# SiyuanHuang95/SUG

Measured on AMD Instinct MI355X. Metric: point-clouds/sec (train step, N=1024), higher is better.
Workload: dtype f32

## Files before the change

sug_amd/csrc/knn_pc.hip:

```cpp
#include <float.h>
#include "common.h"
#include "mfma_tile.h"


namespace {
using namespace sug_tile;

constexpr int SROW = 36;


__device__ __forceinline__ unsigned lds_addr(const float* p) {
  return (unsigned)(uintptr_t)(const __attribute__((address_space(3))) float*)p;
}

template <int KP>
__device__ __forceinline__ void insert_key_hi(int (&L)[KP], int x) {
#pragma unroll
  for (int u = KP - 1; u >= KP / 2; --u) asm volatile("v_med3_i32 %0, %1, %2, %0" : "+v"(L[u]) : "v"(x), "v"(L[u - 1]));
}
template <int KP>
__device__ __forceinline__ void insert_key_lo(int (&L)[KP], int x) {
#pragma unroll
  for (int u = KP / 2 - 1; u >= 1; --u) asm volatile("v_med3_i32 %0, %1, %2, %0" : "+v"(L[u]) : "v"(x), "v"(L[u - 1]));
  asm volatile("v_min_i32 %0, %0, %1" : "+v"(L[0]) : "v"(x));
}

template <int CP>
__device__ __forceinline__ float exact_dot(const float* __restrict__ a, const float* __restrict__ b) {
  float acc = 0.f;
  if constexpr (CP == 4) {
    acc = fmaf(a[0], b[0], acc); acc = fmaf(a[1], b[1], acc); acc = fmaf(a[2], b[2], acc);
  } else {
    for (int e = 0; e < CP; e += 4) {
      const float4 av = *reinterpret_cast<const float4*>(a + e), bv = *reinterpret_cast<const float4*>(b + e);
      acc = fmaf(av.x, bv.x, acc); acc = fmaf(av.y, bv.y, acc); acc = fmaf(av.z, bv.z, acc); acc = fmaf(av.w, bv.w, acc);
    }
  }
  return acc;
}
template <int CP>
__device__ __forceinline__ float exact_norm(const float* __restrict__ r) {
  if constexpr (CP == 4) {
    return sq3(r[0], r[1], r[2]);
  } else {
    constexpr int CH = CP / 8;
    float pc[CH];
#pragma unroll
    for (int c = 0; c < CH; ++c) {
      const float4 a = *reinterpret_cast<const float4*>(r + 8 * c), b = *reinterpret_cast<const float4*>(r + 8 * c + 4);
      float p = __fmul_rn(a.x, a.x);
      p = fmaf(a.y, a.y, p); p = fmaf(a.z, a.z, p); p = fmaf(a.w, a.w, p);
      p = fmaf(b.x, b.x, p); p = fmaf(b.y, b.y, p); p = fmaf(b.z, b.z, p); p = fmaf(b.w, b.w, p);
      pc[c] = p;
    }
#pragma unroll
    for (int o = 1; o < CH; o <<= 1)
#pragma unroll
      for (int c = 0; c < CH; c += 2 * o) pc[c] = pc[c] + pc[c + o];
    return pc[0];
  }
}

template <int CP, int K, int NP, int NC>
__global__ __launch_bounds__(64 * (NP + NC), 2) void knn_pc_kernel(const float* __restrict__ x, int64_t ldx, int B, int N,
                                                                   int k, int32_t* __restrict__ idx, int force) {
  constexpr int RS = CP + 4;
  constexpr int HALF = CP / 2;
  constexpr int NTP = 64 * NP;
  constexpr int QB = 64 * NC;
  constexpr int QP = QB / NP;
  static_assert(QP == 32 || QP == 64, "a producer wave scores one or two 32-query column blocks");
  extern __shared__ __attribute__((aligned(16))) unsigned char smem[];
  float* s_tile = reinterpret_cast<float*>(smem);
  float* s_norm = s_tile + 3 * TJ * RS;
  float* s_score = s_norm + 4 * TJ;

  const int nq = (N + QB - 1) / QB;
  int b, qb;
  if ((B & 7) == 0) {
    const int grp = blockIdx.x / (8 * nq), rem = blockIdx.x % (8 * nq);
    b = grp * 8 + (rem & 7);
    qb = rem >> 3;
  } else {
    b = blockIdx.x / nq;
    qb = blockIdx.x % nq;
  }
  const float* xb = x + (int64_t)b * N * ldx;
  const int wave = (int)(threadIdx.x >> 6);
  const bool producer = wave < NP;
  const int lane = threadIdx.x & 63;
  const int wv = producer ? wave : wave - NP;
  const int ptid = (int)threadIdx.x;
  const int qj = lane & 31, h = lane >> 5;
  const int q0 = qb * QB;

  const int ntile = (N + TJ - 1) / TJ;
  auto tbuf = [&](int t) { return s_tile + (t % 3) * TJ * RS; };
  auto nbuf = [&](int t) { return s_norm + (t % 3) * TJ; };

  if (producer) {
    TileRegs<CP, NTP> tr;
    tile_load<CP, NTP>(tr, xb, ldx, N, 0, ptid);
    float bq0[HALF], bq1[HALF];
    {
      const int r0 = min(q0 + wv * QP + qj, N - 1), r1 = min(q0 + wv * QP + 32 + qj, N - 1);
      const float* p0 = xb + (int64_t)r0 * ldx;
      const float* p1 = xb + (int64_t)r1 * ldx;
      if constexpr (CP == 4) {
        const float x0 = p0[0], y0 = p0[1], z0 = p0[2], x1 = p1[0], y1 = p1[1], z1 = p1[2];
        bq0[0] = -2.f * (h ? y0 : x0); bq0[1] = h ? 0.f : -2.f * z0;
        bq1[0] = -2.f * (h ? y1 : x1); bq1[1] = h ? 0.f : -2.f * z1;
      } else {
#pragma unroll
        for (int g = 0; g < HALF / 4; ++g) {
          const float4 a = *reinterpret_cast<const float4*>(p0 + h * HALF + 4 * g);
          const float4 c = *reinterpret_cast<const float4*>(p1 + h * HALF + 4 * g);
          bq0[4 * g] = -2.f * a.x; bq0[4 * g + 1] = -2.f * a.y; bq0[4 * g + 2] = -2.f * a.z; bq0[4 * g + 3] = -2.f * a.w;
          bq1[4 * g] = -2.f * c.x; bq1[4 * g + 1] = -2.f * c.y; bq1[4 * g + 2] = -2.f * c.z; bq1[4 * g + 3] = -2.f * c.w;
        }
#pragma unroll
        for (int e = 0; e < HALF; e += 2) {
          const auto u = __builtin_amdgcn_permlane32_swap(__float_as_uint(bq0[e]), __float_as_uint(bq0[e + 1]), false, false);
          bq0[e] = __uint_as_float(u[0]); bq0[e + 1] = __uint_as_float(u[1]);
          const auto v = __builtin_amdgcn_permlane32_swap(__float_as_uint(bq1[e]), __float_as_uint(bq1[e + 1]), false, false);
          bq1[e] = __uint_as_float(v[0]); bq1[e + 1] = __uint_as_float(v[1]);
        }
      }
    }
    auto breg = [](int s2) constexpr { return CP == 4 ? s2 : (s2 < HALF / 2 ? 2 * s2 : 2 * (s2 - HALF / 2) + 1); };

    auto produce = [&](int t, int buf, auto&& mid) {
      const float* arow = tbuf(t) + qj * RS + h * HALF;
      f32x16 acc0, acc1;
#pragma unroll
      for (int r = 0; r < 16; ++r) { acc0[r] = 0.f; acc1[r] = 0.f; }
      if constexpr (CP == 4) {
        const float2 a2 = *reinterpret_cast<const float2*>(arow);
        acc0 = __builtin_amdgcn_mfma_f32_32x32x2f32(a2.x, bq0[0], acc0, 0, 0, 0);
        if constexpr (QP == 64) acc1 = __builtin_amdgcn_mfma_f32_32x32x2f32(a2.x, bq1[0], acc1, 0, 0, 0);
        acc0 = __builtin_amdgcn_mfma_f32_32x32x2f32(a2.y, bq0[1], acc0, 0, 0, 0);
        if constexpr (QP == 64) acc1 = __builtin_amdgcn_mfma_f32_32x32x2f32(a2.y, bq1[1], acc1, 0, 0, 0);
        mid();
      } else {
#pragma unroll
        for (int g = 0; g < HALF / 4; ++g) {
          if (g == HALF / 8) mid();
          const float4 a4 = *reinterpret_cast<const float4*>(arow + 4 * g);
          acc0 = __builtin_amdgcn_mfma_f32_32x32x2f32(a4.x, bq0[breg(4 * g + 0)], acc0, 0, 0, 0);
          if constexpr (QP == 64) acc1 = __builtin_amdgcn_mfma_f32_32x32x2f32(a4.x, bq1[breg(4 * g + 0)], acc1, 0, 0, 0);
          acc0 = __builtin_amdgcn_mfma_f32_32x32x2f32(a4.y, bq0[breg(4 * g + 1)], acc0, 0, 0, 0);
          if constexpr (QP == 64) acc1 = __builtin_amdgcn_mfma_f32_32x32x2f32(a4.y, bq1[breg(4 * g + 1)], acc1, 0, 0, 0);
          acc0 = __builtin_amdgcn_mfma_f32_32x32x2f32(a4.z, bq0[breg(4 * g + 2)], acc0, 0, 0, 0);
          if constexpr (QP == 64) acc1 = __builtin_amdgcn_mfma_f32_32x32x2f32(a4.z, bq1[breg(4 * g + 2)], acc1, 0, 0, 0);
          acc0 = __builtin_amdgcn_mfma_f32_32x32x2f32(a4.w, bq0[breg(4 * g + 3)], acc0, 0, 0, 0);
          if constexpr (QP == 64) acc1 = __builtin_amdgcn_mfma_f32_32x32x2f32(a4.w, bq1[breg(4 * g + 3)], acc1, 0, 0, 0);
        }
      }
      float* d0 = s_score + ((buf * QB + wv * QP) + qj) * SROW + 4 * h;
#pragma unroll
      for (int g = 0; g < 4; ++g)
        *reinterpret_cast<float4*>(d0 + 8 * g) = make_float4(acc0[4 * g], acc0[4 * g + 1], acc0[4 * g + 2], acc0[4 * g + 3]);
      if constexpr (QP == 64) {
        float* d1 = d0 + 32 * SROW;
#pragma unroll
        for (int g = 0; g < 4; ++g)
          *reinterpret_cast<float4*>(d1 + 8 * g) = make_float4(acc1[4 * g], acc1[4 * g + 1], acc1[4 * g + 2], acc1[4 * g + 3]);
      }
    };

    tile_store<CP, true, NTP>(tr, tbuf(0), nbuf(0), N, 0, ptid);
    if (ntile > 1) tile_load<CP, NTP>(tr, xb, ldx, N, TJ, ptid);
    __syncthreads();
    produce(0, 0, [] {});
    if (ntile > 1) tile_store<CP, true, NTP>(tr, tbuf(1), nbuf(1), N, TJ, ptid);
    if (ntile > 2) tile_load<CP, NTP>(tr, xb, ldx, N, 2 * TJ, ptid);
    __syncthreads();
    for (int t = 0; t < ntile; ++t) {
      auto stage = [&] {
        if (t + 2 < ntile) tile_store<CP, true, NTP>(tr, tbuf(t + 2), nbuf(t + 2), N, (t + 2) * TJ, ptid);
        if (t + 3 < ntile) tile_load<CP, NTP>(tr, xb, ldx, N, (t + 3) * TJ, ptid);
      };
      if (t + 1 < ntile) produce(t + 1, (t + 1) & 1, [] {});
      stage();
      __syncthreads();
    }
  } else {
    __builtin_amdgcn_s_setprio(1);
    const float ni = exact_norm<CP>(xb + (int64_t)min(q0 + wv * 64 + lane, N - 1) * ldx);

    constexpr int KP = K + 2;
    constexpr int EMPTY = 0x7fffffff;
    int L[KP];
#pragma unroll
    for (int t = 0; t < KP; ++t) L[t] = EMPTY;
    const int q = q0 + wv * 64 + lane;
    const int idb = N > 1 ? 32 - __clz(N - 1) : 0;
    const int idm = (1 << idb) - 1, nidm = ~idm;
    const unsigned FXMAX = (1u << (31 - idb)) - 2u;
    float scale = 1.f, inv_scale = 1.f;
    float thr = -FLT_MAX;

    auto score = [&](float inner, float nj) { return __fsub_rn(__fsub_rn(-nj, inner), ni); };

    __syncthreads();
    __syncthreads();
    for (int t = 0; t < ntile; ++t) {
      const float* srow = s_score + (((t & 1) * QB + wv * 64) + lane) * SROW;
      const float* nrm = nbuf(t);
      unsigned int mask = 0u;
      if (t == 0) {
        float smin = INFINITY;
#pragma unroll
        for (int g = 0; g < 8; ++g) {
          const float4 s4 = *reinterpret_cast<const float4*>(srow + 4 * g);
          const float4 n4 = *reinterpret_cast<const float4*>(nrm + 4 * g);
          const float sx = score(s4.x, n4.x), sy = score(s4.y, n4.y), sz = score(s4.z, n4.z), sw = score(s4.w, n4.w);
          mask = mask + mask + (sx >= thr ? 1u : 0u);
          mask = mask + mask + (sy >= thr ? 1u : 0u);
          mask = mask + mask + (sz >= thr ? 1u : 0u);
          mask = mask + mask + (sw >= thr ? 1u : 0u);
          smin = fminf(smin, sx >= thr ? sx : INFINITY);
          smin = fminf(smin, sy >= thr ? sy : INFINITY);
          smin = fminf(smin, sz >= thr ? sz : INFINITY);
          smin = fminf(smin, sw >= thr ? sw : INFINITY);
        }
        float R = (smin < 0.f && smin > -FLT_MAX) ? -smin : 1.f;
        scale = (float)FXMAX / R;
        inv_scale = R / (float)FXMAX;
        if (!(scale < FLT_MAX) || !(inv_scale > 0.f)) { scale = 1.f; inv_scale = 1.f; }
      } else {
        const float thr2 = thr == -FLT_MAX ? -FLT_MAX : __fsub_rn(__fadd_rn(thr, ni), 2.4e-7f * (fabsf(thr) + fabsf(ni)));
        unsigned int rej = 0u;
#pragma unroll
        for (int g = 0; g < 8; ++g) {
          const float4 s4 = *reinterpret_cast<const float4*>(srow + 4 * g);
          const float4 n4 = *reinterpret_cast<const float4*>(nrm + 4 * g);
          const float wx = __fsub_rn(__fsub_rn(-n4.x, s4.x), thr2), wy = __fsub_rn(__fsub_rn(-n4.y, s4.y), thr2);
          const float wz = __fsub_rn(__fsub_rn(-n4.z, s4.z), thr2), ww = __fsub_rn(__fsub_rn(-n4.w, s4.w), thr2);
          rej = __builtin_amdgcn_alignbit(rej, __float_as_uint(wx), 31);
          rej = __builtin_amdgcn_alignbit(rej, __float_as_uint(wy), 31);
          rej = __builtin_amdgcn_alignbit(rej, __float_as_uint(wz), 31);
          rej = __builtin_amdgcn_alignbit(rej, __float_as_uint(ww), 31);
        }
        mask = ~rej;
      }
      const int pc = __popc(mask);
      unsigned long long cand = ~0ull;
      int nit = 0;
#pragma unroll
      for (int bit = 5; bit >= 0; --bit) {
        const unsigned long long m = __ballot((pc >> bit) & 1) & cand;
        if (m) {
          nit |= 1 << bit;
          cand = m;
        }
      }
      const unsigned srow_a = lds_addr(srow), nrm_a = lds_addr(nrm);
      float dotA, njA, dotB, njB;
      bool vA, vB;
      int cA, cB;
      auto fetch_issue = [&](float& dot, float& nj, bool& valid, int& c) {
        valid = mask != 0u;
        c = valid ? __builtin_clz(mask) : 0;
        mask &= ~(0x80000000u >> c);
        asm volatile("ds_read_b32 %0, %2\n\tds_read_b32 %1, %3" : "=&v"(dot), "=&v"(nj) : "v"(srow_a + 4u * c), "v"(nrm_a + 4u * c));
      };
      auto fetch_finish = [&](float& dot, float& nj, bool valid, int c, int& key_out) {
        asm volatile("s_waitcnt lgkmcnt(2)" : "+v"(dot), "+v"(nj));
        const unsigned fx = min(__float2uint_rz(-score(dot, nj) * scale), FXMAX);
        key_out = valid ? (int)((fx << idb) | (unsigned)(t * TJ + c)) : EMPTY;
      };
      int key_cur, key_nxt;
      fetch_issue(dotA, njA, vA, cA);
      fetch_issue(dotB, njB, vB, cB);
      fetch_finish(dotA, njA, vA, cA, key_cur);
      for (int it = 0; it < nit; it += 2) {
        fetch_issue(dotA, njA, vA, cA);
        insert_key_hi<KP>(L, key_cur);
        fetch_finish(dotB, njB, vB, cB, key_nxt);
        insert_key_lo<KP>(L, key_cur);
        if (it + 1 < nit) {
          fetch_issue(dotB, njB, vB, cB);
          insert_key_hi<KP>(L, key_nxt);
          fetch_finish(dotA, njA, vA, cA, key_cur);
          insert_key_lo<KP>(L, key_nxt);
        }
      }
      asm volatile("s_waitcnt lgkmcnt(0)" : "+v"(dotA), "+v"(njA), "+v"(dotB), "+v"(njB));
      const int lk = L[KP - 1];
      thr = lk == EMPTY ? -FLT_MAX : -((float)((lk >> idb) + 3) * inv_scale * 1.000002f);
      __syncthreads();
    }

    bool amb = false;
#pragma unroll
    for (int u = 0; u < K; ++u) amb |= ((L[u] ^ L[u + 1]) & nidm) == 0 && L[u] != EMPTY;
    bool rescan = amb && ((L[K - 1] ^ L[KP - 1]) & nidm) == 0 && L[KP - 1] != EMPTY;
    if (force >= 1) amb = true;
    if (force >= 2) rescan = true;
    if (q >= N) amb = rescan = false;
    int32_t* o = idx + ((int64_t)b * N + (q < N ? q : 0)) * k;
    if (q < N && !amb) {
#pragma unroll
      for (int t = 0; t < K; ++t)
        if (t < k) o[t] = L[t] == EMPTY ? q : (L[t] & idm);
    }
    if (__ballot(amb) != 0ull) {
      int* s_keys = reinterpret_cast<int*>(s_score + (0 * QB + wv * 64) * SROW);
      float* s_fv = s_score + (1 * QB + wv * 64) * SROW;
#pragma unroll
      for (int t = 0; t < KP; ++t) s_keys[lane * KP + t] = L[t];
      unsigned long long todo = __ballot(amb && !rescan);
      while (todo) {
        const int ql = __builtin_ctzll(todo);
        todo &= todo - 1;
        const int qi = q0 + wv * 64 + ql;
        const float niq = __shfl(ni, ql);
        const int key = lane < KP ? s_keys[ql * KP + lane] : EMPTY;
        const bool has = key != EMPTY;
        const int j = has ? (key & idm) : 0;
        const float* xq = xb + (int64_t)qi * ldx;
        const float* xj = xb + (int64_t)j * ldx;
        const float dj = exact_dot<CP>(xj, xq);
        const float nj = exact_norm<CP>(xj);
        const float sc = has ? __fsub_rn(__fsub_rn(-nj, __fmul_rn(-2.0f, dj)), niq) : -INFINITY;
        int rank = 0;
#pragma unroll
        for (int v = 0; v < KP; ++v) {
          const float sv = __int_as_float(__builtin_amdgcn_readlane(__float_as_int(sc), v));
          const int jv = __builtin_amdgcn_readlane(has ? j : 0x7fffffff, v);
          rank += (sv > sc || (sv == sc && jv < j)) ? 1 : 0;
        }
        const int nhas = __popcll(__ballot(has));
        int32_t* oq = idx + ((int64_t)b * N + qi) * k;
        if (has && rank < k) oq[rank] = j;
        if (lane < k && lane >= nhas) oq[lane] = qi;
      }
      if (rescan) {
        int* s_fid = s_keys;
        const float* xq = xb + (int64_t)q * ldx;
        for (int t = 0; t < K; ++t) { s_fv[t * 64 + lane] = -INFINITY; s_fid[t * 64 + lane] = q; }
        for (int j = 0; j < N; ++j) {
          const float* xj = xb + (int64_t)j * ldx;
          const float sc = __fsub_rn(__fsub_rn(-exact_norm<CP>(xj), __fmul_rn(-2.0f, exact_dot<CP>(xj, xq))), ni);
          if (sc > s_fv[(K - 1) * 64 + lane]) {
            int u = K - 1;
            while (u > 0 && sc > s_fv[(u - 1) * 64 + lane]) {
              s_fv[u * 64 + lane] = s_fv[(u - 1) * 64 + lane];
              s_fid[u * 64 + lane] = s_fid[(u - 1) * 64 + lane];
              --u;
            }
            s_fv[u * 64 + lane] = sc;
            s_fid[u * 64 + lane] = j;
          }
        }
        for (int t = 0; t < K; ++t)
          if (t < k) o[t] = s_fid[t * 64 + lane];
      }
    }
  }
}

template <int CP, int K, int NP, int NC>
int launch_pc_form(const float* x, int64_t ldx, int B, int N, int k, int32_t* idx, hipStream_t st) {
  constexpr int RS = CP + 4;
  constexpr int QB = 64 * NC;
  const size_t sh = (size_t)(3 * TJ * RS + 4 * TJ + 2 * QB * SROW) * sizeof(float);
  static SugLdsOptIn note;
  if (int rc = sug_allow_dynamic_lds(note, &knn_pc_kernel<CP, K, NP, NC>, (int)sh, "sug_knn(mfma, producer/consumer)")) return rc;
  dim3 grid(sug_divup(N, QB) * B);
  const char* fe = getenv("SUG_KNN_FORCE");
  hipLaunchKernelGGL((knn_pc_kernel<CP, K, NP, NC>), grid, dim3(64 * (NP + NC)), sh, st, x, ldx, B, N, k, idx, fe ? atoi(fe) : 0);
  SUG_LAUNCH_CHECK("sug_knn(mfma, producer/consumer)");
  return SUG_OK;
}

template <int CP, int K>
int launch_pc(const float* x, int64_t ldx, int B, int N, int k, int32_t* idx, hipStream_t st) {
  static const int forced = getenv("SUG_KNN_PW") ? atoi(getenv("SUG_KNN_PW")) : 0;
  const int ncu = sug_cu_count();
  const int64_t grid4 = (int64_t)B * sug_divup(N, 256);
  const bool small = 2 * grid4 <= ncu;
  const int form = (forced == 4 || forced == 44) ? 44 : (forced == 2 || forced == 22) ? 22 : forced == 42 ? 42
                   : !small ? 44 : (CP >= 64 ? 42 : 22);
  if (form == 22) return launch_pc_form<CP, K, 2, 2>(x, ldx, B, N, k, idx, st);
  if (form == 42) return launch_pc_form<CP, K, 4, 2>(x, ldx, B, N, k, idx, st);
  return launch_pc_form<CP, K, 4, 4>(x, ldx, B, N, k, idx, st);
}

template <int K>
int dispatch_pc(const float* x, int64_t ldx, int B, int N, int C, int k, int32_t* idx, hipStream_t st) {
  if (C == 3) return launch_pc<4, K>(x, ldx, B, N, k, idx, st);
  if (C == 64) return launch_pc<64, K>(x, ldx, B, N, k, idx, st);
  return launch_pc<128, K>(x, ldx, B, N, k, idx, st);
}

}

int sug_knn_pc_supported(const float* x, int64_t ldx, int C, int k) {
  if (k > 20) return 0;
  if (C == 3) return 1;
  if (C != 64 && C != 128) return 0;
  return ((uintptr_t)x % 16 == 0) && (ldx % 4 == 0);
}

int sug_knn_pc(const float* x, int64_t ldx, int B, int N, int C, int k, int32_t* idx, hipStream_t st) {
  if (k <= 16) return dispatch_pc<16>(x, ldx, B, N, C, k, idx, st);
  return dispatch_pc<20>(x, ldx, B, N, C, k, idx, st);
}
```

Measured before the change: 13610.

## Fold neighbour norm into MFMA accumulation and use ballot-driven consumer loop

Adds an MF variant in which the producer scales the query by +2 and folds the negated neighbour norm into the score accumulator with one extra rank-1 MFMA. Consumers then read only the fused score, dropping the per-candidate norm LDS loads and one subtraction. The consumer also preloads the score row into registers, and the popcount/ballot bit-search for the iteration count is replaced by a ballot-terminated while loop. This shifts a small amount of work onto the producer's matrix cores and changes the floating-point rounding order of the score, which could affect tie or threshold behaviour.

```diff
diff --git a/sug_amd/csrc/knn_pc.hip b/sug_amd/csrc/knn_pc.hip
--- a/sug_amd/csrc/knn_pc.hip
+++ b/sug_amd/csrc/knn_pc.hip
@@ -61,7 +61,7 @@
   }
 }
 
-template <int CP, int K, int NP, int NC>
+template <int CP, int K, int NP, int NC, int MF>
 __global__ __launch_bounds__(64 * (NP + NC), 2) void knn_pc_kernel(const float* __restrict__ x, int64_t ldx, int B, int N,
                                                                    int k, int32_t* __restrict__ idx, int force) {
   constexpr int RS = CP + 4;
@@ -99,6 +99,7 @@
   auto nbuf = [&](int t) { return s_norm + (t % 3) * TJ; };
 
   if (producer) {
+    constexpr float QS = MF == 0 ? -2.f : 2.f;
     TileRegs<CP, NTP> tr;
     tile_load<CP, NTP>(tr, xb, ldx, N, 0, ptid);
     float bq0[HALF], bq1[HALF];
@@ -108,15 +109,15 @@
       const float* p1 = xb + (int64_t)r1 * ldx;
       if constexpr (CP == 4) {
         const float x0 = p0[0], y0 = p0[1], z0 = p0[2], x1 = p1[0], y1 = p1[1], z1 = p1[2];
-        bq0[0] = -2.f * (h ? y0 : x0); bq0[1] = h ? 0.f : -2.f * z0;
-        bq1[0] = -2.f * (h ? y1 : x1); bq1[1] = h ? 0.f : -2.f * z1;
+        bq0[0] = QS * (h ? y0 : x0); bq0[1] = h ? 0.f : QS * z0;
+        bq1[0] = QS * (h ? y1 : x1); bq1[1] = h ? 0.f : QS * z1;
       } else {
 #pragma unroll
         for (int g = 0; g < HALF / 4; ++g) {
           const float4 a = *reinterpret_cast<const float4*>(p0 + h * HALF + 4 * g);
           const float4 c = *reinterpret_cast<const float4*>(p1 + h * HALF + 4 * g);
-          bq0[4 * g] = -2.f * a.x; bq0[4 * g + 1] = -2.f * a.y; bq0[4 * g + 2] = -2.f * a.z; bq0[4 * g + 3] = -2.f * a.w;
-          bq1[4 * g] = -2.f * c.x; bq1[4 * g + 1] = -2.f * c.y; bq1[4 * g + 2] = -2.f * c.z; bq1[4 * g + 3] = -2.f * c.w;
+          bq0[4 * g] = QS * a.x; bq0[4 * g + 1] = QS * a.y; bq0[4 * g + 2] = QS * a.z; bq0[4 * g + 3] = QS * a.w;
+          bq1[4 * g] = QS * c.x; bq1[4 * g + 1] = QS * c.y; bq1[4 * g + 2] = QS * c.z; bq1[4 * g + 3] = QS * c.w;
         }
 #pragma unroll
         for (int e = 0; e < HALF; e += 2) {
@@ -155,6 +156,11 @@
           acc0 = __builtin_amdgcn_mfma_f32_32x32x2f32(a4.w, bq0[breg(4 * g + 3)], acc0, 0, 0, 0);
           if constexpr (QP == 64) acc1 = __builtin_amdgcn_mfma_f32_32x32x2f32(a4.w, bq1[breg(4 * g + 3)], acc1, 0, 0, 0);
         }
+      }
+      if constexpr (MF == 1) {
+        const float nj = h == 0 ? nbuf(t)[qj] : 0.f, m1 = h == 0 ? -1.f : 0.f;
+        acc0 = __builtin_amdgcn_mfma_f32_32x32x2f32(nj, m1, acc0, 0, 0, 0);
+        if constexpr (QP == 64) acc1 = __builtin_amdgcn_mfma_f32_32x32x2f32(nj, m1, acc1, 0, 0, 0);
       }
       float* d0 = s_score + ((buf * QB + wv * QP) + qj) * SROW + 4 * h;
 #pragma unroll
@@ -201,6 +207,7 @@
     float thr = -FLT_MAX;
 
     auto score = [&](float inner, float nj) { return __fsub_rn(__fsub_rn(-nj, inner), ni); };
+    auto score_u = [&](float u) { return __fsub_rn(u, ni); };
 
     __syncthreads();
     __syncthreads();
@@ -213,8 +220,13 @@
 #pragma unroll
         for (int g = 0; g < 8; ++g) {
           const float4 s4 = *reinterpret_cast<const float4*>(srow + 4 * g);
-          const float4 n4 = *reinterpret_cast<const float4*>(nrm + 4 * g);
-          const float sx = score(s4.x, n4.x), sy = score(s4.y, n4.y), sz = score(s4.z, n4.z), sw = score(s4.w, n4.w);
+          float sx, sy, sz, sw;
+          if constexpr (MF == 0) {
+            const float4 n4 = *reinterpret_cast<const float4*>(nrm + 4 * g);
+            sx = score(s4.x, n4.x); sy = score(s4.y, n4.y); sz = score(s4.z, n4.z); sw = score(s4.w, n4.w);
+          } else {
+            sx = score_u(s4.x); sy = score_u(s4.y); sz = score_u(s4.z); sw = score_u(s4.w);
+          }
           mask = mask + mask + (sx >= thr ? 1u : 0u);
           mask = mask + mask + (sy >= thr ? 1u : 0u);
           mask = mask + mask + (sz >= thr ? 1u : 0u);
@@ -231,12 +243,21 @@
       } else {
         const float thr2 = thr == -FLT_MAX ? -FLT_MAX : __fsub_rn(__fadd_rn(thr, ni), 2.4e-7f * (fabsf(thr) + fabsf(ni)));
         unsigned int rej = 0u;
+        float4 sv[8];
+#pragma unroll
+        for (int g = 0; g < 8; ++g) sv[g] = *reinterpret_cast<const float4*>(srow + 4 * g);
+        __builtin_amdgcn_sched_barrier(0);
 #pragma unroll
         for (int g = 0; g < 8; ++g) {
-          const float4 s4 = *reinterpret_cast<const float4*>(srow + 4 * g);
-          const float4 n4 = *reinterpret_cast<const float4*>(nrm + 4 * g);
-          const float wx = __fsub_rn(__fsub_rn(-n4.x, s4.x), thr2), wy = __fsub_rn(__fsub_rn(-n4.y, s4.y), thr2);
-          const float wz = __fsub_rn(__fsub_rn(-n4.z, s4.z), thr2), ww = __fsub_rn(__fsub_rn(-n4.w, s4.w), thr2);
+          const float4 s4 = sv[g];
+          float wx, wy, wz, ww;
+          if constexpr (MF == 0) {
+            const float4 n4 = *reinterpret_cast<const float4*>(nrm + 4 * g);
+            wx = __fsub_rn(__fsub_rn(-n4.x, s4.x), thr2); wy = __fsub_rn(__fsub_rn(-n4.y, s4.y), thr2);
+            wz = __fsub_rn(__fsub_rn(-n4.z, s4.z), thr2); ww = __fsub_rn(__fsub_rn(-n4.w, s4.w), thr2);
+          } else {
+            wx = __fsub_rn(s4.x, thr2); wy = __fsub_rn(s4.y, thr2); wz = __fsub_rn(s4.z, thr2); ww = __fsub_rn(s4.w, thr2);
+          }
           rej = __builtin_amdgcn_alignbit(rej, __float_as_uint(wx), 31);
           rej = __builtin_amdgcn_alignbit(rej, __float_as_uint(wy), 31);
           rej = __builtin_amdgcn_alignbit(rej, __float_as_uint(wz), 31);
@@ -244,47 +265,43 @@
         }
         mask = ~rej;
       }
-      const int pc = __popc(mask);
-      unsigned long long cand = ~0ull;
-      int nit = 0;
-#pragma unroll
-      for (int bit = 5; bit >= 0; --bit) {
-        const unsigned long long m = __ballot((pc >> bit) & 1) & cand;
-        if (m) {
-          nit |= 1 << bit;
-          cand = m;
-        }
-      }
       const unsigned srow_a = lds_addr(srow), nrm_a = lds_addr(nrm);
-      float dotA, njA, dotB, njB;
+      float dotA, njA = 0.f, dotB, njB = 0.f;
       bool vA, vB;
       int cA, cB;
       auto fetch_issue = [&](float& dot, float& nj, bool& valid, int& c) {
         valid = mask != 0u;
         c = valid ? __builtin_clz(mask) : 0;
         mask &= ~(0x80000000u >> c);
-        asm volatile("ds_read_b32 %0, %2\n\tds_read_b32 %1, %3" : "=&v"(dot), "=&v"(nj) : "v"(srow_a + 4u * c), "v"(nrm_a + 4u * c));
+        if constexpr (MF == 0)
+          asm volatile("ds_read_b32 %0, %2\n\tds_read_b32 %1, %3" : "=&v"(dot), "=&v"(nj) : "v"(srow_a + 4u * c), "v"(nrm_a + 4u * c));
+        else
+          asm volatile("ds_read_b32 %0, %1" : "=&v"(dot) : "v"(srow_a + 4u * c));
       };
       auto fetch_finish = [&](float& dot, float& nj, bool valid, int c, int& key_out) {
-        asm volatile("s_waitcnt lgkmcnt(2)" : "+v"(dot), "+v"(nj));
-        const unsigned fx = min(__float2uint_rz(-score(dot, nj) * scale), FXMAX);
+        if constexpr (MF == 0) asm volatile("s_waitcnt lgkmcnt(2)" : "+v"(dot), "+v"(nj));
+        else asm volatile("s_waitcnt lgkmcnt(1)" : "+v"(dot));
+        const float sc = MF == 0 ? score(dot, nj) : score_u(dot);
+        const unsigned fx = min(__float2uint_rz(-sc * scale), FXMAX);
         key_out = valid ? (int)((fx << idb) | (unsigned)(t * TJ + c)) : EMPTY;
       };
       int key_cur, key_nxt;
       fetch_issue(dotA, njA, vA, cA);
       fetch_issue(dotB, njB, vB, cB);
       fetch_finish(dotA, njA, vA, cA, key_cur);
-      for (int it = 0; it < nit; it += 2) {
+      bool more = __ballot(vA) != 0ull;
+      while (more) {
+        const bool more1 = __ballot(vB) != 0ull;
         fetch_issue(dotA, njA, vA, cA);
         insert_key_hi<KP>(L, key_cur);
         fetch_finish(dotB, njB, vB, cB, key_nxt);
         insert_key_lo<KP>(L, key_cur);
-        if (it + 1 < nit) {
-          fetch_issue(dotB, njB, vB, cB);
-          insert_key_hi<KP>(L, key_nxt);
-          fetch_finish(dotA, njA, vA, cA, key_cur);
-          insert_key_lo<KP>(L, key_nxt);
-        }
+        if (!more1) break;
+        more = __ballot(vA) != 0ull;
+        fetch_issue(dotB, njB, vB, cB);
+        insert_key_hi<KP>(L, key_nxt);
+        fetch_finish(dotA, njA, vA, cA, key_cur);
+        insert_key_lo<KP>(L, key_nxt);
       }
       asm volatile("s_waitcnt lgkmcnt(0)" : "+v"(dotA), "+v"(njA), "+v"(dotB), "+v"(njB));
       const int lk = L[KP - 1];
@@ -361,18 +378,24 @@
   }
 }
 
-template <int CP, int K, int NP, int NC>
+template <int CP, int K, int NP, int NC, int MF>
 int launch_pc_form(const float* x, int64_t ldx, int B, int N, int k, int32_t* idx, hipStream_t st) {
   constexpr int RS = CP + 4;
   constexpr int QB = 64 * NC;
   const size_t sh = (size_t)(3 * TJ * RS + 4 * TJ + 2 * QB * SROW) * sizeof(float);
   static SugLdsOptIn note;
-  if (int rc = sug_allow_dynamic_lds(note, &knn_pc_kernel<CP, K, NP, NC>, (int)sh, "sug_knn(mfma, producer/consumer)")) return rc;
+  if (int rc = sug_allow_dynamic_lds(note, &knn_pc_kernel<CP, K, NP, NC, MF>, (int)sh, "sug_knn(mfma, producer/consumer)")) return rc;
   dim3 grid(sug_divup(N, QB) * B);
   const char* fe = getenv("SUG_KNN_FORCE");
-  hipLaunchKernelGGL((knn_pc_kernel<CP, K, NP, NC>), grid, dim3(64 * (NP + NC)), sh, st, x, ldx, B, N, k, idx, fe ? atoi(fe) : 0);
+  hipLaunchKernelGGL((knn_pc_kernel<CP, K, NP, NC, MF>), grid, dim3(64 * (NP + NC)), sh, st, x, ldx, B, N, k, idx, fe ? atoi(fe) : 0);
   SUG_LAUNCH_CHECK("sug_knn(mfma, producer/consumer)");
   return SUG_OK;
+}
+
+template <int CP, int K, int NP, int NC>
+int launch_pc_chain(int mf, const float* x, int64_t ldx, int B, int N, int k, int32_t* idx, hipStream_t st) {
+  if (mf == 0) return launch_pc_form<CP, K, NP, NC, 0>(x, ldx, B, N, k, idx, st);
+  return launch_pc_form<CP, K, NP, NC, 1>(x, ldx, B, N, k, idx, st);
 }
 
 template <int CP, int K>
@@ -383,9 +406,11 @@
   const bool small = 2 * grid4 <= ncu;
   const int form = (forced == 4 || forced == 44) ? 44 : (forced == 2 || forced == 22) ? 22 : forced == 42 ? 42
                    : !small ? 44 : (CP >= 64 ? 42 : 22);
-  if (form == 22) return launch_pc_form<CP, K, 2, 2>(x, ldx, B, N, k, idx, st);
-  if (form == 42) return launch_pc_form<CP, K, 4, 2>(x, ldx, B, N, k, idx, st);
-  return launch_pc_form<CP, K, 4, 4>(x, ldx, B, N, k, idx, st);
+  static const int mf_forced = getenv("SUG_KNN_MFMA") ? atoi(getenv("SUG_KNN_MFMA")) : -1;
+  const int mf = (mf_forced == 0 || mf_forced == 1) ? mf_forced : (form == 22 && CP >= 64 ? 0 : 1);
+  if (form == 22) return launch_pc_chain<CP, K, 2, 2>(mf, x, ldx, B, N, k, idx, st);
+  if (form == 42) return launch_pc_chain<CP, K, 4, 2>(mf, x, ldx, B, N, k, idx, st);
+  return launch_pc_chain<CP, K, 4, 4>(mf, x, ldx, B, N, k, idx, st);
 }
 
 template <int K>
```

Measured after the change: 13710, median of 6. No clear change (+0.8%).
